# MAC-VO/MAC-VO

Hardware: AMD Instinct MI355X
Metric: stereo frames/sec at 640x480 (hot path: cost volume + lookup, keypoint selection, covariance, PGO) (higher is better)
Workload: dtype f32 via f16x2 (volume: fp32 operands row-scaled by powers of two and split into two fp16 pieces, three products, fp32 accumulate, scales undone exactly) + f32 (lookup/covariance) + f64 (PGO)

## Files before the change

mac-vo_amd/csrc/frontend_ops.hip:

```cpp
#include "common.h"
#include "randperm_dev.h"
#include "kp_draw_dev.h"
#include "match_cov_dev.h"
#include "pose_apply_dev.h"
#include "obs_filter_dev.h"
#include <math.h>

namespace {

__global__ __launch_bounds__(256) void frontend_epilogue_kernel(
    const float* __restrict__ flow, const float* __restrict__ logcov, int cov_is_log, int plane, float bl_fx,
    float bl_fx_sq, float* __restrict__ disparity, float* __restrict__ disparity_cov, float* __restrict__ depth,
    float* __restrict__ depth_cov, uint8_t* __restrict__ bad_mask, float* __restrict__ match_flow,
    float* __restrict__ match_cov) {
    MV_CHAIN_KERNEL_PRIO();
    const size_t lo = (size_t)blockIdx.y * plane;
    flow += 4 * lo; logcov += 4 * lo;
    if (disparity) disparity += lo;
    if (disparity_cov) disparity_cov += lo;
    if (depth) depth += lo;
    if (depth_cov) depth_cov += lo;
    if (bad_mask) bad_mask += lo;
    if (match_flow) match_flow += 2 * lo;
    if (match_cov) match_cov += 3 * lo;
// ... 170 lines not shown
    const float u = kp_uv[2 * n], v = kp_uv[2 * n + 1], d = depth_vals[(size_t)n * depth_stride];
    const float p[3] = {d, ((u - cx) * d) / fx, ((v - cy) * d) / fy};
    if (pos_Tc) { pos_Tc[3 * n] = p[0]; pos_Tc[3 * n + 1] = p[1]; pos_Tc[3 * n + 2] = p[2]; }
    if (pos_Tw) {
        float r[3];
        quat_act_f32(q, p, r);
        pos_Tw[3 * n] = r[0] + t[0]; pos_Tw[3 * n + 1] = r[1] + t[1]; pos_Tw[3 * n + 2] = r[2] + t[2];
    }
}

__global__ __launch_bounds__(256) void pose_apply_kernel(const float* __restrict__ pose, const float* __restrict__ pos_Tc,
                                                         const double* __restrict__ cov, int cap, mvLaneCounts cnt,
                                                         float* __restrict__ pos_Tw, double* __restrict__ rot,
                                                         double* __restrict__ cov_rot) {
    const int n = blockIdx.x * blockDim.x + threadIdx.x;
    const int lane = blockIdx.y;
    const int N = cnt.n[lane];
    {
        const size_t ln = (size_t)lane * cap;
        pose += 7 * lane;
        if (pos_Tc) pos_Tc += 3 * ln;
        if (pos_Tw) pos_Tw += 3 * ln;
        if (cov) cov += 9 * ln;
        if (cov_rot) cov_rot += 9 * ln;
        if (rot) rot += 9 * lane;
    }
    double R[9];
    mv_pose_rotation(pose, R);
    if (n == 0 && rot) {
#pragma unroll
        for (int i = 0; i < 9; ++i) rot[i] = R[i];
    }
    if (n >= N) return;
    mv_pose_apply_row(pose, R, n, pos_Tc, cov, pos_Tw, cov_rot);
}

__global__ __launch_bounds__(256) void map_points_kernel(const int64_t* __restrict__ uv, int N,
                                                          const float* __restrict__ depth, const float* __restrict__ depth_cov,
                                                          const float* __restrict__ image, int H, int W, float fx, float fy,
                                                          float cx, float cy, const float* __restrict__ pose,
                                                          float match_cov_default, float* __restrict__ out_uv,
                                                          float* __restrict__ out_d, float* __restrict__ out_sdd,
                                                          float* __restrict__ out_sigma, float* __restrict__ out_Tc,
                                                          float* __restrict__ out_Tw, uint8_t* __restrict__ out_color) {
    const int n = blockIdx.x * blockDim.x + threadIdx.x;
    if (n >= N) return;
    const int u = (int)uv[2 * n], v = (int)uv[2 * n + 1];
    const bool ok = u >= 0 && u < W && v >= 0 && v < H;
    const int i = ok ? v * W + u : 0;
    const float d = depth[i];
    const float uf = (float)u, vf = (float)v;
    out_uv[2 * n] = uf;
    out_uv[2 * n + 1] = vf;
    if (out_d) out_d[n] = d;
    if (out_sdd) out_sdd[n] = depth_cov ? depth_cov[i] : -1.f;
    if (out_sigma) { out_sigma[3 * n] = match_cov_default; out_sigma[3 * n + 1] = match_cov_default; out_sigma[3 * n + 2] = 0.f; }
    const float pc[3] = {d, ((uf - cx) * d) / fx, ((vf - cy) * d) / fy};
    if (out_Tc) { out_Tc[3 * n] = pc[0]; out_Tc[3 * n + 1] = pc[1]; out_Tc[3 * n + 2] = pc[2]; }
    if (out_Tw) {
        const float q[4] = {pose[3], pose[4], pose[5], pose[6]};
        float r[3];
        quat_act_f32(q, pc, r);
        out_Tw[3 * n] = r[0] + pose[0]; out_Tw[3 * n + 1] = r[1] + pose[1]; out_Tw[3 * n + 2] = r[2] + pose[2];
    }
    if (out_color && image) {
        const size_t plane = (size_t)H * W;
#pragma unroll
        for (int c = 0; c < 3; ++c) {
            const float x = image[c * plane + i] * 255.f;
            out_color[3 * n + c] = (uint8_t)(int)x;
        }
    }
}

__global__ __launch_bounds__(256) void obs_filter_kernel(const uint8_t* __restrict__ inbound,
                                                         const double* __restrict__ cov1,
                                                         const double* __restrict__ cov2,
                                                         const float* __restrict__ vals, int flags,
                                                         float min_depth, float max_depth, int cap, mvLaneCounts cnt,
                                                         uint8_t* __restrict__ valid, int32_t* __restrict__ count) {
    obs_filter_body(inbound, cov1, cov2, vals, flags, min_depth, max_depth, cap, cnt.n[blockIdx.x], blockIdx.x, gridDim.x, valid, count);
}

struct DrawArgs {
    const int32_t* count;
    int count_stride;
    float nomatch_c;
    const uint32_t* state_in;
    uint32_t* state_out;
    int k;
    int32_t cov_mods;
    int64_t* out_perm;
    int32_t* out_live;
};
struct DrawLds {
    mvrp::Scratch s;
    int32_t head[mvrp::NBUCKET];
    int32_t out[mvrp::MAX_HEAD];
};
template <int PM, int MODEL = MV_COV_MATCH, bool MODS = false, bool NOMATCH = false>
__global__ __launch_bounds__(256) void backend_front_kernel(const int32_t* __restrict__ cand, size_t cand_lane_stride, const int64_t* __restrict__ perm,
                                                            PermArg pa, int cap, mvLaneCounts cnt, int64_t* out_uv, TrackArgs a, float fx, float fy,
                                                            float cx, float cy, float* pos_Tc, const float* depth_map0, const float* depth_map1,
                                                            double* out_cov0, double* out_cov1, mvMatchCovParams cp, DrawArgs da) {
    __shared__ __attribute__((aligned(16))) char draw_raw[PM == 2 ? sizeof(DrawLds) : PM == 4 ? sizeof(mvkp::Scratch) : 16];
    DrawLds& D = *reinterpret_cast<DrawLds*>(draw_raw);
    const int lane = threadIdx.x & 63;
    const int n = blockIdx.x * 4 + (threadIdx.x >> 6);
    const int set = blockIdx.y, pl = blockIdx.z;
    int N;
    if constexpr (PM == 2) {
        const int64_t n_cand = da.count[(size_t)pl * da.count_stride];
        const bool adv = blockIdx.x == 0 && blockIdx.y == 0;
        N = mv_randperm_head_wg(da.state_in + (size_t)pl * mvrp::MT_STRIDE, adv ? da.state_out + (size_t)pl * mvrp::MT_STRIDE : nullptr, n_cand, da.k,
                                D.out, D.s, D.head);
        __syncthreads();
        if (adv) {
            for (int i = threadIdx.x; i < N; i += 256) da.out_perm[(size_t)pl * cap + i] = D.out[i];
            if (threadIdx.x == 0) { da.out_live[2 * pl] = N; da.out_live[2 * pl + 1] = (int32_t)n_cand; }
        }
    } else if constexpr (PM == 3) {
        if (da.count) {
            const int c = da.count[(size_t)pl * da.count_stride];
            N = c < 0 ? 0 : (c > cap ? cap : c);
        } else {
            N = cnt.n[pl];
        }
        if (da.out_live && blockIdx.x == 0 && blockIdx.y == 0 && threadIdx.x == 0) { da.out_live[2 * pl] = N; da.out_live[2 * pl + 1] = N; }
    } else if constexpr (PM == 4) {
        N = cnt.n[pl];
        const bool adv = blockIdx.x == 0 && blockIdx.y == 0;
        mv_kp_random_wg(da.state_in + (size_t)pl * mvrp::MT_STRIDE, adv ? da.state_out + (size_t)pl * mvrp::MT_STRIDE : nullptr, da.k,
                        *reinterpret_cast<mvkp::Scratch*>(draw_raw));
    } else {
        N = cnt.n[pl];
    }
    if (n < N) {
        int u0, v0;
        if constexpr (PM <= 2) {
            const int32_t* cand_l = cand + (size_t)pl * cand_lane_stride;
            const long pi = PM == 2 ? (long)D.out[n] : PM == 1 ? (long)pa.idx[n] : (long)perm[(size_t)pl * cap + n];
            const int lin = cand_l[pi];
            u0 = lin % a.W;
            v0 = lin / a.W;
        } else if constexpr (PM == 3) {
            const int64_t* kp = perm + 2 * ((size_t)pl * cap + n);
            u0 = (int)kp[0];
            v0 = (int)kp[1];
        } else if constexpr (PM == 4) {
            mvkp::row_of(reinterpret_cast<mvkp::Scratch*>(draw_raw)->w, da.k, n, a.H, a.W, pa.idx[0], u0, v0);
        } else {
            mvkp::grid_row(mvkp::Grid{pa.idx[0], 0, pa.idx[1], pa.idx[2], pa.idx[3]}, n, u0, v0);
        }
        TrackArgs al = a;
        track_lane_offsets(al, pl, cap);
        const size_t ln = (size_t)pl * cap;
        float u, v, suu, svv, suv;
        if (set == 0) {
            if (lane == 0) {
                if (PM != 3 || out_uv != perm) {
                    out_uv[2 * (ln + n) + 0] = u0;
                    out_uv[2 * (ln + n) + 1] = v0;
                }
                kp_track_one(n, u0, v0, al.match_flow, al.match_cov, al.depth0, al.disp0, al.sdisp0, al.sdd0, al.depth1, al.disp1, al.sdisp1, al.sdd1,
                             al.H, al.W, al.edge, al.match_cov_default, al.out_kp0, al.out_kp1, al.out_inbound, al.out_vals, (size_t)gridDim.z * cap,
                             nullptr, nullptr);
                al.out_sigma0[3 * n + 2] = 0.f;
                const float uf = (float)u0, vf = (float)v0, d = al.out_vals[n];
                float* pt = pos_Tc + 3 * (ln + n);
                pt[0] = d;
                pt[1] = ((uf - cx) * d) / fx;
                pt[2] = ((vf - cy) * d) / fy;
            }
            u = (float)u0; v = (float)v0;
            suu = a.match_cov_default; svv = a.match_cov_default; suv = 0.f;
        } else {
            const int plane = al.H * al.W;
            const bool ok0 = u0 >= 0 && u0 < al.W && v0 >= 0 && v0 < al.H;
            const int i0 = ok0 ? v0 * al.W + u0 : 0;
            u = (float)u0 + al.match_flow[i0];
            v = (float)v0 + al.match_flow[plane + i0];
            if constexpr (NOMATCH) {
                if (lane == 0) { al.out_sigma1[3 * n] = -1.f; al.out_sigma1[3 * n + 1] = -1.f; al.out_sigma1[3 * n + 2] = -1.f; }
                const bool inb = ok0 && (u < (float)(al.W - al.edge)) && (u > (float)al.edge) && (v < (float)(al.H - al.edge)) && (v > (float)al.edge);
                const bool have_var = al.sdd1 != nullptr;
                const float var = have_var && inb ? al.sdd1[(int)v * al.W + (int)u] : 0.f;
                const mvcov::CovSet S1{depth_map1, nullptr, nullptr, nullptr, nullptr, out_cov1, nullptr, nullptr};
                mvcov::match_cov_wave_vals<MODEL, MODS, true>(S1, cp, cap, pl, n, u, v, da.nomatch_c, da.nomatch_c, 0.f, da.cov_mods, a.sdd1, var, have_var);
                return;
            }
            suu = al.match_cov ? al.match_cov[i0] : -1.f;
            svv = al.match_cov ? al.match_cov[plane + i0] : -1.f;
            suv = al.match_cov ? al.match_cov[2 * plane + i0] : -1.f;
            if (lane == 0) al.out_sigma1[3 * n + 2] = suv;
        }
        const mvcov::CovSet S{set ? depth_map1 : depth_map0, nullptr, set ? a.out_sigma1 : a.out_sigma0, nullptr, nullptr, set ? out_cov1 : out_cov0,
                              nullptr, nullptr};
        if constexpr (MODEL == MV_COV_MATCH && !MODS)
            mvcov::match_cov_wave_vals(S, cp, cap, pl, n, u, v, suu, svv, suv);
        else
            mvcov::match_cov_wave_vals<MODEL, MODS>(S, cp, cap, pl, n, u, v, suu, svv, suv, da.cov_mods, set ? a.sdd1 : a.sdd0);
    }
}

template <int PM, typename... Args>
void launch_backend_front(int model, int32_t mods, bool nomatch, float nomatch_c, dim3 grid, hipStream_t st, DrawArgs da, Args... args) {
    const bool m = mods != 0;
    da.cov_mods = mods;
    if constexpr (PM >= 3) if (nomatch) {
        da.nomatch_c = nomatch_c;
        if (model == MV_COV_MATCH && !m)
            hipLaunchKernelGGL((backend_front_kernel<PM, MV_COV_MATCH, false, true>), grid, dim3(256), 0, st, args..., da);
        else if (model == MV_COV_MATCH)
            hipLaunchKernelGGL((backend_front_kernel<PM, MV_COV_MATCH, true, true>), grid, dim3(256), 0, st, args..., da);
        else if (model == MV_COV_GMM && !m)
            hipLaunchKernelGGL((backend_front_kernel<PM, MV_COV_GMM, false, true>), grid, dim3(256), 0, st, args..., da);
        else if (model == MV_COV_GMM)
            hipLaunchKernelGGL((backend_front_kernel<PM, MV_COV_GMM, true, true>), grid, dim3(256), 0, st, args..., da);
        else if (!m)
            hipLaunchKernelGGL((backend_front_kernel<PM, MV_COV_NONE, false, true>), grid, dim3(256), 0, st, args..., da);
        else
            hipLaunchKernelGGL((backend_front_kernel<PM, MV_COV_NONE, true, true>), grid, dim3(256), 0, st, args..., da);
        return;
    }
    if (model == MV_COV_MATCH && !m)
        hipLaunchKernelGGL((backend_front_kernel<PM>), grid, dim3(256), 0, st, args..., da);
    else if (model == MV_COV_MATCH)
        hipLaunchKernelGGL((backend_front_kernel<PM, MV_COV_MATCH, true>), grid, dim3(256), 0, st, args..., da);
    else if (model == MV_COV_GMM && !m)
        hipLaunchKernelGGL((backend_front_kernel<PM, MV_COV_GMM, false>), grid, dim3(256), 0, st, args..., da);
    else if (model == MV_COV_GMM)
        hipLaunchKernelGGL((backend_front_kernel<PM, MV_COV_GMM, true>), grid, dim3(256), 0, st, args..., da);
    else if (!m)
        hipLaunchKernelGGL((backend_front_kernel<PM, MV_COV_NONE, false>), grid, dim3(256), 0, st, args..., da);
    else
        hipLaunchKernelGGL((backend_front_kernel<PM, MV_COV_NONE, true>), grid, dim3(256), 0, st, args..., da);
}

template <typename... Args>
void launch_backend_front_pm(int pm, Args... args) {
    switch (pm) {
        case 1: return launch_backend_front<1>(args...);
        case 0: return launch_backend_front<0>(args...);
        case 2: return launch_backend_front<2>(args...);
        case 3: return launch_backend_front<3>(args...);
        case 4: return launch_backend_front<4>(args...);
        case 5: return launch_backend_front<5>(args...);
    }
}

}

extern "C" int mv_frontend_epilogue_lanes(const float* flow, const float* logcov, int cov_is_log, int H, int W,
                                          float bl_fx, float bl_fx_sq, float* disparity, float* disparity_cov,
                                          float* depth, float* depth_cov, uint8_t* bad_mask, float* match_flow,
                                          float* match_cov, int lanes, mvStream_t stream) {
    MV_CHECK_ARG(flow && H > 0 && W > 0 && lanes >= 1 && lanes <= MV_MAX_LANES);
    const int plane = H * W;
    const int blocks = min(mv_ceil_div(plane, 256), 2048);
    const bool no_d = !disparity_cov && !depth_cov, no_m = match_flow && !match_cov;
    MV_CHECK_ARG(logcov || (no_d && !match_cov));
    if (!logcov || no_d || no_m) {
        const dim3 grid(blocks, lanes);
#define MV_EPI_PARTIAL(D, M)                                                                                                                             \
    hipLaunchKernelGGL((frontend_epilogue_partial_kernel<D, M>), grid, dim3(256), 0, (hipStream_t)stream, flow, logcov, cov_is_log, plane, bl_fx, bl_fx_sq, \
                       disparity, disparity_cov, depth, depth_cov, bad_mask, match_flow, match_cov)
        if (!logcov || (no_d && !match_cov)) MV_EPI_PARTIAL(false, false);
        else if (no_d) MV_EPI_PARTIAL(false, true);
        else MV_EPI_PARTIAL(true, false);
#undef MV_EPI_PARTIAL
        return mv_launch_status();
    }
    hipLaunchKernelGGL(frontend_epilogue_kernel, dim3(blocks, lanes), dim3(256), 0, (hipStream_t)stream, flow, logcov,
                       cov_is_log, plane, bl_fx, bl_fx_sq, disparity, disparity_cov, depth, depth_cov, bad_mask,
                       match_flow, match_cov);
    return mv_launch_status();
}

extern "C" int mv_frontend_epilogue(const float* flow, const float* logcov, int cov_is_log, int H, int W,
                                    float bl_fx, float bl_fx_sq, float* disparity, float* disparity_cov, float* depth,
                                    float* depth_cov, uint8_t* bad_mask, float* match_flow, float* match_cov,
                                    mvStream_t stream) {
    return mv_frontend_epilogue_lanes(flow, logcov, cov_is_log, H, W, bl_fx, bl_fx_sq, disparity, disparity_cov, depth,
                                      depth_cov, bad_mask, match_flow, match_cov, 1, stream);
// ... 276 lines not shown
```

mac-vo_amd/csrc/match_cov_dev.h:

```cpp
#pragma once
#include "common.h"
#include <math.h>

namespace mvcov {

constexpr int MAX_K = 31;
constexpr int MAX_TAPS_PER_LANE = (MAX_K * MAX_K + 63) / 64;

__device__ __forceinline__ float clamp_min_nanprop(float x, float m) { return (x < m) ? m : x; }

struct CovSet {
    const float* depth_map;
    const float* kp_uv;
    float* flow_cov;
    const float* depth_cov;
    const double* rot;
    double* out_cov;
    double* out_cov_rot;
    float* out_stats;
};

__device__ __forceinline__ void apply_modifiers(double c[9], int32_t mods) {
#pragma unroll
    for (int s = 0; s < 4; ++s) {
        const int k = (mods >> (4 * s)) & 15;
        if (k == MV_COVMOD_DIAG) {
            c[1] = 0.0; c[2] = 0.0; c[3] = 0.0; c[5] = 0.0; c[6] = 0.0; c[7] = 0.0;
        } else if (k == MV_COVMOD_NORMALIZE) {
            const double det = (c[0] * (c[4] * c[8] - c[5] * c[7]) - c[1] * (c[3] * c[8] - c[5] * c[6])) + c[2] * (c[3] * c[7] - c[4] * c[6]);
#pragma unroll
            for (int i = 0; i < 9; ++i) c[i] = c[i] / det;
        }
    }
}

template <bool MODS>
__device__ __forceinline__ void store_cov(double c[9], int32_t mods, const double* rot, double* out_cov, double* out_cov_rot, float* out_stats,
                                          int n, float mu, float var) {
    if constexpr (MODS) apply_modifiers(c, mods);
    double* o = out_cov + (size_t)n * 9;
#pragma unroll
    for (int i = 0; i < 9; ++i) o[i] = c[i];
    if (out_cov_rot && rot) {
        double R[9], t[9];
#pragma unroll
        for (int i = 0; i < 9; ++i) R[i] = rot[i];
#pragma unroll
        for (int i = 0; i < 3; ++i)
#pragma unroll
            for (int j = 0; j < 3; ++j)
                t[3 * i + j] = (R[3 * i] * c[j] + R[3 * i + 1] * c[3 + j]) + R[3 * i + 2] * c[6 + j];
        double* orot = out_cov_rot + (size_t)n * 9;
#pragma unroll
        for (int i = 0; i < 3; ++i)
#pragma unroll
            for (int j = 0; j < 3; ++j)
                orot[3 * i + j] = (t[3 * i] * R[3 * j] + t[3 * i + 1] * R[3 * j + 1]) + t[3 * i + 2] * R[3 * j + 2];
    }
    if (out_stats) {
        out_stats[2 * n] = mu;
        out_stats[2 * n + 1] = var;
    }
}

template <int MODEL = MV_COV_MATCH, bool MODS = false, bool NOMATCH = false>
__device__ __forceinline__ void match_cov_wave_vals(const CovSet& S, const mvMatchCovParams& p, int cap, int pl, int n, float u, float v,
                                                    float suu, float svv, float suv, int32_t mods = 0,
                                                    const float* depth_cov_map_all = nullptr ,
                                                    float var_given = 0.f, bool have_var = false ) {
    const int lane = threadIdx.x & 63;
    const size_t ln = (size_t)pl * cap;
    const float* __restrict__ depth_map = S.depth_map + (size_t)pl * p.H * p.W;
    float* __restrict__ flow_cov = S.flow_cov + 3 * ln;
    const float* __restrict__ depth_cov = S.depth_cov ? S.depth_cov + ln : nullptr;
    const double* __restrict__ rot = S.rot ? S.rot + 9 * pl : nullptr;
    double* __restrict__ out_cov = S.out_cov + 9 * ln;
    double* __restrict__ out_cov_rot = S.out_cov_rot ? S.out_cov_rot + 9 * ln : nullptr;
    float* __restrict__ out_stats = S.out_stats ? S.out_stats + 2 * ln : nullptr;

    if constexpr (MODEL == MV_COV_NONE) {
        if (lane == 0) {
            if constexpr (!NOMATCH) {
                flow_cov[3 * n] = suu;
                flow_cov[3 * n + 1] = svv;
            }
            double c[9] = {1.0, 0.0, 0.0, 0.0, 1.0, 0.0, 0.0, 0.0, 1.0};
            store_cov<MODS>(c, mods, rot, out_cov, out_cov_rot, out_stats, n, __builtin_nanf(""), __builtin_nanf(""));
        }
        return;
    }
    const float* __restrict__ depth_cov_map = MODEL == MV_COV_GMM ? depth_cov_map_all + (size_t)pl * p.H * p.W : nullptr;

    const int iu = (int)u, iv = (int)v;
    if constexpr (!NOMATCH) {
        suu = clamp_min_nanprop(suu, p.min_flow_cov_sq);
        svv = clamp_min_nanprop(svv, p.min_flow_cov_sq);
        if (lane == 0) {
            flow_cov[3 * n] = suu;
            flow_cov[3 * n + 1] = svv;
        }
    }
    bool patch_var;
    if constexpr (NOMATCH) patch_var = !have_var; else patch_var = p.use_patch_var;

    const float det = suu * svv - suv * suv;
    const float m00 = -0.5f * (svv / det), m01 = -0.5f * (-suv / det), m11 = -0.5f * (suu / det);
    const float cnorm = (2.f * 3.14159265358979323846f) * sqrtf(det);

    const int K = p.kernel_size, h = K >> 1, taps = K * K;
    float z[MAX_TAPS_PER_LANE], kv[MAX_TAPS_PER_LANE];
    float zc[MODEL == MV_COV_GMM ? MAX_TAPS_PER_LANE : 1];
    float ksum = 0.f;
#pragma unroll
    for (int r = 0; r < MAX_TAPS_PER_LANE; ++r) {
        const int idx = r * 64 + lane;
        z[r] = 0.f;
        kv[r] = 0.f;
        if constexpr (MODEL == MV_COV_GMM) zc[r] = 0.f;
        if (idx < taps) {
            const int a = idx / K, b = idx - a * K;
            int yy = iv + (a - h), xx = iu + (b - h);
            yy = min(max(yy, 0), p.H - 1);
            xx = min(max(xx, 0), p.W - 1);
            z[r] = depth_map[yy * p.W + xx];
            if constexpr (MODEL == MV_COV_GMM) zc[r] = depth_cov_map[yy * p.W + xx] + z[r] * z[r];
            const float x0 = (float)(a - h), x1 = (float)(b - h);
            const float q = (x0 * m00) * x0 + 2.f * ((x0 * m01) * x1) + (x1 * m11) * x1;
            kv[r] = expf(q) / cnorm;
            ksum += kv[r];
        }
    }
    ksum = wave_sum(ksum);

    float mu = 0.f, var;
    if constexpr (MODEL == MV_COV_GMM) {
        float psum = 0.f;
#pragma unroll
        for (int r = 0; r < MAX_TAPS_PER_LANE; ++r) {
            kv[r] = kv[r] / ksum;
            if (kv[r] < 1e-3f) kv[r] = 0.f;
            psum += kv[r];
        }
        psum = wave_sum(psum);
        float e2 = 0.f;
#pragma unroll
        for (int r = 0; r < MAX_TAPS_PER_LANE; ++r) {
            kv[r] = kv[r] / psum;
            mu += z[r] * kv[r];
            e2 += zc[r] * kv[r];
        }
        mu = wave_sum(mu);
        e2 = wave_sum(e2);
        if constexpr (NOMATCH) var = patch_var ? (e2 - mu * mu) / 2.f : var_given;
        else var = patch_var ? (e2 - mu * mu) / 2.f : depth_cov[n];
    } else {
#pragma unroll
        for (int r = 0; r < MAX_TAPS_PER_LANE; ++r) {
            kv[r] = kv[r] / ksum;
            mu += kv[r] * z[r];
        }
        mu = wave_sum(mu);

        if (patch_var) {
            var = 0.f;
#pragma unroll
            for (int r = 0; r < MAX_TAPS_PER_LANE; ++r) {
                const float d = z[r] - mu;
                var += kv[r] * (d * d);
            }
            var = wave_sum(var);
        } else {
            if constexpr (NOMATCH) var = var_given; else var = depth_cov[n];
        }
        var = clamp_min_nanprop(var, p.min_depth_cov);
    }

    if (lane == 0) {
        const float du = u - p.cx, dv = v - p.cy;
        const float fx2 = p.fx * p.fx, fy2 = p.fy * p.fy, fxy = p.fx * p.fy;
        const float d2 = mu * mu;
        const float sxx = (((du * du) * var) + (d2 * suu) + (suu * var)) / fx2;
        const float syy = (((dv * dv) * var) + (d2 * svv) + (svv * var)) / fy2;
        const float szz = var;
        const float sxy = (((du * dv) * var) + (d2 + var) * suv) / fxy;
        const float sxz = (var * du) / p.fx;
        const float syz = (var * dv) / p.fy;
        double c[9] = {szz, sxz, syz, sxz, sxx, sxy, syz, sxy, syy};
        if constexpr (MODS) apply_modifiers(c, mods);
        double* o = out_cov + (size_t)n * 9;
#pragma unroll
        for (int i = 0; i < 9; ++i) o[i] = c[i];
        if (out_cov_rot && rot) {
            double R[9], t[9];
#pragma unroll
            for (int i = 0; i < 9; ++i) R[i] = rot[i];
#pragma unroll
            for (int i = 0; i < 3; ++i)
#pragma unroll
                for (int j = 0; j < 3; ++j)
                    t[3 * i + j] = (R[3 * i] * c[j] + R[3 * i + 1] * c[3 + j]) + R[3 * i + 2] * c[6 + j];
            double* orot = out_cov_rot + (size_t)n * 9;
#pragma unroll
            for (int i = 0; i < 3; ++i)
#pragma unroll
                for (int j = 0; j < 3; ++j)
                    orot[3 * i + j] = (t[3 * i] * R[3 * j] + t[3 * i + 1] * R[3 * j + 1]) + t[3 * i + 2] * R[3 * j + 2];
        }
        if (out_stats) {
            out_stats[2 * n] = mu;
            out_stats[2 * n + 1] = var;
        }
    }
}


template <int MODEL = MV_COV_MATCH, bool MODS = false>
__device__ __forceinline__ void match_cov_wave(const CovSet& S, const mvMatchCovParams& p, int cap, int pl, int n, int32_t mods = 0,
                                               const float* depth_cov_map = nullptr) {
    const size_t ln = (size_t)pl * cap;
    const float* __restrict__ kp_uv = S.kp_uv + 2 * ln;
    const float* __restrict__ flow_cov = S.flow_cov + 3 * ln;
    match_cov_wave_vals<MODEL, MODS>(S, p, cap, pl, n, kp_uv[2 * n], kp_uv[2 * n + 1], flow_cov[3 * n], flow_cov[3 * n + 1], flow_cov[3 * n + 2],
                                     mods, depth_cov_map);
}

template <int MODEL, bool MODS>
__device__ __forceinline__ void match_cov_wave_nomatch(const CovSet& S, const mvMatchCovParams& p, int cap, int pl, int n, float c, int32_t mods,
                                                       const float* depth_cov_map) {
    const size_t ln = (size_t)pl * cap;
    const float* __restrict__ kp_uv = S.kp_uv + 2 * ln;
    const bool have = S.depth_cov != nullptr;
    const float var = have ? S.depth_cov[ln + n] : 0.f;
    match_cov_wave_vals<MODEL, MODS, true>(S, p, cap, pl, n, kp_uv[2 * n], kp_uv[2 * n + 1], c, c, 0.f, mods, depth_cov_map, var, have);
}

}
```

mac-vo_amd/csrc/randperm.hip:

```cpp
#include "common.h"
#include "randperm_dev.h"
#include <vector>

int mv_randperm_heads_emulated_state(uint32_t* state, const int64_t* n, int calls, int k, int threads, int64_t* out);

namespace {

__global__ __launch_bounds__(1024) void randperm_head_kernel(uint32_t* __restrict__ state, const int32_t* __restrict__ n_dev, int n_stride, int k, int cap,
                                                             int64_t* __restrict__ out, int32_t* __restrict__ n_sel, int nsel_stride) {
    __shared__ mvrp::Scratch s;
    __shared__ int32_t head[mvrp::NBUCKET];
    const int l = blockIdx.x;
    uint32_t* const st = state + (size_t)l * mvrp::MT_STRIDE;
    const int m = mv_randperm_head_wg(st, st, (int64_t)n_dev[(size_t)l * n_stride], k, out + (size_t)l * cap, s, head);
    if (threadIdx.x == 0) n_sel[(size_t)l * nsel_stride] = m;
}

}

extern "C" int mv_randperm_state_words(void) { return mvrp::MT_STRIDE; }
extern "C" int mv_randperm_max_head(void) { return mvrp::MAX_HEAD; }

extern "C" int mv_mt19937_seed(uint64_t seed, uint32_t* state_host) {
    MV_CHECK_ARG(state_host);
    mvrp::mt_seed((uint32_t)(seed & 0xffffffffull), state_host);
    return MV_OK;
}

extern "C" int mv_randperm_head_lanes(uint32_t* state, const int32_t* n_dev, int n_stride, int lanes, int k, int cap, int64_t* out_perm, int32_t* out_n_sel,
                                      int n_sel_stride, mvStream_t stream) {
    MV_CHECK_ARG(state && n_dev && out_perm && out_n_sel && lanes >= 1 && n_stride >= 1 && n_sel_stride >= 1);
    MV_CHECK_ARG(k >= 0 && k <= cap);
    if (k > mvrp::MAX_HEAD) return MV_ERR_UNSUPPORTED;
    hipLaunchKernelGGL(randperm_head_kernel, dim3(lanes), dim3(1024), 0, (hipStream_t)stream, state, n_dev, n_stride, k, cap, out_perm, out_n_sel, n_sel_stride);
    return mv_launch_status();
}

extern "C" int mv_randperm_heads_emulated(uint64_t seed, const int64_t* n, int calls, int k, int threads, int64_t* out) {
    std::vector<uint32_t> state(mvrp::MT_STRIDE);
    mvrp::mt_seed((uint32_t)(seed & 0xffffffffull), state.data());
    return mv_randperm_heads_emulated_state(state.data(), n, calls, k, threads, out);
}

int mv_randperm_heads_emulated_state(uint32_t* state, const int64_t* n, int calls, int k, int threads, int64_t* out) {
    using namespace mvrp;
    MV_CHECK_ARG(state && n && out && calls >= 0 && k >= 0 && threads >= 1 && threads <= 4096);
    if (k > MAX_HEAD) return MV_ERR_UNSUPPORTED;
    std::vector<int32_t> head(NBUCKET);
    Scratch* s = new Scratch;
    const int nt = threads;
#define MV_RP_ALL(call) for (int tid = 0; tid < nt; ++tid) { call; }
    for (int c = 0; c < calls; ++c) {
        MV_CHECK_ARG(n[c] >= 0 && n[c] < ((int64_t)1 << 31));
        const Plan pl = plan_of(n[c], k);
        MV_RP_ALL(phase_clear(head.data(), tid, nt));
        if (pl.advance > 0) {
            for (int i = 0; i < MT_N; ++i) s->mt[0][i] = state[i];
            int pos = (int)state[MT_N], cur = 0;
            int64_t produced = 0, rem = pl.advance;
            while (rem > 0) {
                if (pos == MT_N) {
                    MV_RP_ALL(phase_step(s->mt[cur], s->mt[cur ^ 1], tid, nt));
                    cur ^= 1;
                    pos = 0;
                }
                const int take = (int)(rem < MT_N - pos ? rem : MT_N - pos);
                if (produced < pl.swaps) MV_RP_ALL(phase_draws(s->mt[cur], pos, take, produced, pl, s->t, tid, nt));
                pos += take;
                produced += take;
                rem -= take;
            }
            for (int i = 0; i < MT_N; ++i) state[i] = s->mt[cur][i];
            state[MT_N] = (uint32_t)pos;
        }
        MV_RP_ALL(phase_insert(*s, head.data(), pl, tid, nt));
        MV_RP_ALL(phase_link(*s, head.data(), pl, tid, nt));
        MV_RP_ALL(phase_emit(*s, pl, out + (size_t)c * k, tid, nt));
    }
#undef MV_RP_ALL
    delete s;
    return MV_OK;
}
```

mac-vo_amd/csrc/randperm_dev.h:

```cpp
#pragma once
#include <stdint.h>

#if defined(__HIPCC__)
#define MV_RP_FN __host__ __device__ __forceinline__
#else
#define MV_RP_FN inline
#endif

namespace mvrp {

constexpr int MT_N = 624;
constexpr int MT_STRIDE = 640;
constexpr int MAX_HEAD = 512;
constexpr int NBUCKET = 1024;

struct Scratch {
    uint32_t mt[2][MT_N];
    int32_t t[MAX_HEAD], nxt[MAX_HEAD], ptr[MAX_HEAD], hit[MAX_HEAD];
};

MV_RP_FN uint32_t mt_f(uint32_t a, uint32_t b) {
    const uint32_t y = (a & 0x80000000u) | (b & 0x7fffffffu);
    return (y >> 1) ^ ((b & 1u) ? 0x9908b0dfu : 0u);
}
// ... 17 lines not shown

inline void mt_seed(uint32_t seed, uint32_t* state ) {
    state[0] = seed;
    for (int i = 1; i < MT_N; ++i) state[i] = 1812433253u * (state[i - 1] ^ (state[i - 1] >> 30)) + (uint32_t)i;
    state[MT_N] = MT_N;
    for (int i = MT_N + 1; i < MT_STRIDE; ++i) state[i] = 0;
}

struct Plan {
    int64_t n;
    int swaps, m;
    int64_t advance;
};
MV_RP_FN Plan plan_of(int64_t n, int k) {
    Plan p;
    p.n = n;
    p.m = (int)(n < k ? (n < 0 ? 0 : n) : k);
    p.swaps = n >= 1 ? (int)(k < n - 1 ? k : n - 1) : 0;
    p.advance = n >= 1 ? n - 1 : 0;
    return p;
}

MV_RP_FN void phase_step(const uint32_t* o, uint32_t* nw, int tid, int nt) {
    for (int k = tid; k < MT_N; k += nt) nw[k] = mt_step_word(o, k);
}

MV_RP_FN void phase_draws(const uint32_t* x, int pos, int take, int64_t produced, const Plan& pl, int32_t* t, int tid, int nt) {
    for (int j = tid; j < take; j += nt) {
        const int64_t g = produced + j;
        if (g >= pl.swaps) break;
        t[g] = (int32_t)(g + (int64_t)(mt_temper(x[pos + j]) % (uint32_t)(pl.n - g)));
    }
}

MV_RP_FN void phase_clear(int32_t* head, int tid, int nt) {
    for (int b = tid; b < NBUCKET; b += nt) head[b] = -1;
}

#if defined(__HIP_DEVICE_COMPILE__)
#define MV_RP_XCHG(p, v) atomicExch((p), (v))
#else
static inline int32_t mv_rp_xchg_host(int32_t* p, int32_t v) { const int32_t o = *p; *p = v; return o; }
#define MV_RP_XCHG(p, v) mv_rp_xchg_host((p), (v))
#endif

MV_RP_FN void phase_insert(Scratch& s, int32_t* head, const Plan& pl, int tid, int nt) {
    for (int j = tid; j < pl.m; j += nt) {
        if (j < pl.swaps) s.nxt[j] = MV_RP_XCHG(&head[s.t[j] & (NBUCKET - 1)], j);
        else s.t[j] = j;
    }
}

MV_RP_FN int32_t prev_of(const Scratch& s, const int32_t* head, int i, int32_t p) {
    int32_t best = -1;
    for (int32_t e = head[p & (NBUCKET - 1)]; e >= 0; e = s.nxt[e])
        if (e < i && s.t[e] == p && e > best) best = e;
    return best;
}

MV_RP_FN void phase_link(Scratch& s, const int32_t* head, const Plan& pl, int tid, int nt) {
    for (int i = tid; i < pl.m; i += nt) {
        s.ptr[i] = prev_of(s, head, i, i);
        s.hit[i] = s.t[i] == i ? -2 : prev_of(s, head, i, s.t[i]);
    }
}

MV_RP_FN int32_t root_of(const Scratch& s, int32_t i) {
    while (s.ptr[i] >= 0) i = s.ptr[i];
    return i;
}

template <typename T>
MV_RP_FN void phase_emit(const Scratch& s, const Plan& pl, T* out, int tid, int nt) {
    for (int i = tid; i < pl.m; i += nt) {
        const int32_t h = s.hit[i];
        out[i] = (T)(h == -2 ? root_of(s, i) : (h >= 0 ? root_of(s, h) : s.t[i]));
    }
}

}

#if defined(__HIPCC__)
template <typename T>
__device__ __forceinline__ int mv_randperm_head_wg(const uint32_t* __restrict__ state_in, uint32_t* state_out, int64_t n, int k, T* out, mvrp::Scratch& s,
                                                   int32_t* head) {
    using namespace mvrp;
    const int tid = threadIdx.x, nt = blockDim.x;
    const Plan pl = plan_of(n, k);
    phase_clear(head, tid, nt);
    if (pl.advance > 0 || state_out) {
        for (int i = tid; i < MT_N; i += nt) s.mt[0][i] = state_in[i];
        int pos = (int)state_in[MT_N];
        __syncthreads();
        int cur = 0;
        int64_t produced = 0;
        const int64_t total = state_out ? pl.advance : (int64_t)pl.swaps;
        int64_t rem = total;
        while (rem > 0) {
            if (pos == MT_N) {
                phase_step(s.mt[cur], s.mt[cur ^ 1], tid, nt);
                __syncthreads();
                cur ^= 1;
                pos = 0;
            }
            const int take = (int)(rem < MT_N - pos ? rem : MT_N - pos);
            if (produced < pl.swaps) phase_draws(s.mt[cur], pos, take, produced, pl, s.t, tid, nt);
            pos += take;
            produced += take;
            rem -= take;
        }
        if (state_out) {
            for (int i = tid; i < MT_N; i += nt) state_out[i] = s.mt[cur][i];
            if (tid == 0) state_out[MT_N] = (uint32_t)pos;
        }
    }
    __syncthreads();
    phase_insert(s, head, pl, tid, nt);
    __syncthreads();
    phase_link(s, head, pl, tid, nt);
    __syncthreads();
    phase_emit(s, pl, out, tid, nt);
    return pl.m;
}
#endif
```

Baseline: 7564.

## Issue front-kernel pixel and window loads early and spread them across lanes

In the backend front kernel, lane 0 no longer does a serial chain of pixel reads through kp_track_one. Each lane now loads one source or tracked pixel value, and the values are broadcast with readlane. The covariance window taps and Gaussian weights move into separate request and weights phases that run before the per-set branching, so global loads are in flight earlier. The randperm head also prefetches the Mersenne Twister state and count into registers before the plan is computed. The aim is to shorten the latency-bound dependent load chain, at the cost of more registers and duplicated inbound logic. A standalone timing probe script is added as well.

```diff
diff --git a/mac-vo_amd/csrc/frontend_ops.hip b/mac-vo_amd/csrc/frontend_ops.hip
--- a/mac-vo_amd/csrc/frontend_ops.hip
+++ b/mac-vo_amd/csrc/frontend_ops.hip
@@ -276,6 +276,27 @@
     obs_filter_body(inbound, cov1, cov2, vals, flags, min_depth, max_depth, cap, cnt.n[blockIdx.x], blockIdx.x, gridDim.x, valid, count);
 }
 
+enum { FS_FLOW_U, FS_FLOW_V, FS_SUU, FS_SVV, FS_SUV, FS_DEPTH, FS_DISP, FS_SDISP, FS_SDD };
+__device__ __forceinline__ float lane_value(float x, int k) { return __int_as_float(__builtin_amdgcn_readlane(__float_as_int(x), k)); }
+__device__ __forceinline__ float front_source_pixel(const TrackArgs& al, int lane, int i0, int plane) {
+    const float* p = al.match_flow;
+    int off = i0;
+    if (lane == FS_FLOW_V) off = plane + i0;
+    if (lane >= FS_SUU && lane <= FS_SUV && al.match_cov) { p = al.match_cov; off = (lane - FS_SUU) * plane + i0; }
+    if (lane == FS_DEPTH) p = al.depth0;
+    if (lane == FS_DISP && al.disp0) p = al.disp0;
+    if (lane == FS_SDISP && al.sdisp0) p = al.sdisp0;
+    if (lane == FS_SDD && al.sdd0) p = al.sdd0;
+    return p[off];
+}
+__device__ __forceinline__ float front_tracked_pixel(const TrackArgs& al, int lane, int i1) {
+    const float* p = al.depth1;
+    if (lane == 1 && al.disp1) p = al.disp1;
+    if (lane == 2 && al.sdisp1) p = al.sdisp1;
+    if (lane == 3 && al.sdd1) p = al.sdd1;
+    return p[i1];
+}
+
 struct DrawArgs {
     const int32_t* count;
     int count_stride;
@@ -304,10 +325,10 @@
     const int set = blockIdx.y, pl = blockIdx.z;
     int N;
     if constexpr (PM == 2) {
-        const int64_t n_cand = da.count[(size_t)pl * da.count_stride];
+        int64_t n_cand;
         const bool adv = blockIdx.x == 0 && blockIdx.y == 0;
-        N = mv_randperm_head_wg(da.state_in + (size_t)pl * mvrp::MT_STRIDE, adv ? da.state_out + (size_t)pl * mvrp::MT_STRIDE : nullptr, n_cand, da.k,
-                                D.out, D.s, D.head);
+        N = mv_randperm_head_wg(da.state_in + (size_t)pl * mvrp::MT_STRIDE, adv ? da.state_out + (size_t)pl * mvrp::MT_STRIDE : nullptr,
+                                da.count + (size_t)pl * da.count_stride, n_cand, da.k, D.out, D.s, D.head);
         __syncthreads();
         if (adv) {
             for (int i = threadIdx.x; i < N; i += 256) da.out_perm[(size_t)pl * cap + i] = D.out[i];
@@ -349,51 +370,82 @@
         TrackArgs al = a;
         track_lane_offsets(al, pl, cap);
         const size_t ln = (size_t)pl * cap;
-        float u, v, suu, svv, suv;
+        const int plane = al.H * al.W;
+        const bool ok0 = u0 >= 0 && u0 < al.W && v0 >= 0 && v0 < al.H;
+        const int i0 = ok0 ? v0 * al.W + u0 : 0;
+        const float x0 = front_source_pixel(al, lane, i0, plane);
+        if constexpr (NOMATCH) if (set == 1) {
+            const float u = (float)u0 + lane_value(x0, FS_FLOW_U);
+            const float v = (float)v0 + lane_value(x0, FS_FLOW_V);
+            const bool inb = ok0 && (u < (float)(al.W - al.edge)) && (u > (float)al.edge) && (v < (float)(al.H - al.edge)) && (v > (float)al.edge);
+            const bool have_var = al.sdd1 != nullptr;
+            const float var1 = (have_var ? al.sdd1 : al.depth1)[inb ? (int)v * al.W + (int)u : 0];
+            mvcov::CovWindow<MODEL> w;
+            mvcov::cov_window_request<MODEL>(depth_map1, a.sdd1, cp, pl, u, v, w);
+            float suu = da.nomatch_c, svv = da.nomatch_c;
+            mvcov::cov_window_weights<MODEL, true>(cp, suu, svv, 0.f, w);
+            if (lane == 0) { al.out_sigma1[3 * n] = -1.f; al.out_sigma1[3 * n + 1] = -1.f; al.out_sigma1[3 * n + 2] = -1.f; }
+            const float var = have_var && inb ? var1 : 0.f;
+            const mvcov::CovSet S1{depth_map1, nullptr, nullptr, nullptr, nullptr, out_cov1, nullptr, nullptr};
+            mvcov::match_cov_wave_finish<MODEL, MODS, true>(S1, cp, cap, pl, n, u, v, suu, svv, 0.f, da.cov_mods, var, have_var, w);
+            return;
+        }
+        float u = (float)u0, v = (float)v0;
+        float suu = a.match_cov_default, svv = a.match_cov_default, suv = 0.f;
+        if (set == 1) {
+            u = (float)u0 + lane_value(x0, FS_FLOW_U);
+            v = (float)v0 + lane_value(x0, FS_FLOW_V);
+            suu = al.match_cov ? lane_value(x0, FS_SUU) : -1.f;
+            svv = al.match_cov ? lane_value(x0, FS_SVV) : -1.f;
+            suv = al.match_cov ? lane_value(x0, FS_SUV) : -1.f;
+        }
+        mvcov::CovWindow<MODEL> w;
+        mvcov::cov_window_request<MODEL>(set ? depth_map1 : depth_map0, set ? a.sdd1 : a.sdd0, cp, pl, u, v, w);
+        mvcov::cov_window_weights<MODEL, false>(cp, suu, svv, suv, w);
         if (set == 0) {
+            const float u1 = (float)u0 + lane_value(x0, FS_FLOW_U);
+            const float v1 = (float)v0 + lane_value(x0, FS_FLOW_V);
+            const bool inb = ok0 && (u1 < (float)(al.W - al.edge)) && (u1 > (float)al.edge) && (v1 < (float)(al.H - al.edge)) && (v1 > (float)al.edge);
+            const int i1 = inb ? (int)v1 * al.W + (int)u1 : 0;
+            const float x1 = front_tracked_pixel(al, lane, i1);
+            const float d = lane_value(x0, FS_DEPTH);
+            const float t_disp = lane_value(x0, FS_DISP), t_sdisp = lane_value(x0, FS_SDISP), t_sdd = lane_value(x0, FS_SDD);
+            const float m_uu = lane_value(x0, FS_SUU), m_vv = lane_value(x0, FS_SVV), m_uv = lane_value(x0, FS_SUV);
+            const float d1 = lane_value(x1, 0), t_disp1 = lane_value(x1, 1), t_sdisp1 = lane_value(x1, 2), t_sdd1 = lane_value(x1, 3);
             if (lane == 0) {
                 if (PM != 3 || out_uv != perm) {
                     out_uv[2 * (ln + n) + 0] = u0;
                     out_uv[2 * (ln + n) + 1] = v0;
                 }
-                kp_track_one(n, u0, v0, al.match_flow, al.match_cov, al.depth0, al.disp0, al.sdisp0, al.sdd0, al.depth1, al.disp1, al.sdisp1, al.sdd1,
-                             al.H, al.W, al.edge, al.match_cov_default, al.out_kp0, al.out_kp1, al.out_inbound, al.out_vals, (size_t)gridDim.z * cap,
-                             nullptr, nullptr);
+                if (al.out_kp0) { al.out_kp0[2 * n] = (float)u0; al.out_kp0[2 * n + 1] = (float)v0; }
+                al.out_kp1[2 * n] = u1;
+                al.out_kp1[2 * n + 1] = v1;
+                al.out_inbound[n] = inb;
+                const size_t vs = (size_t)gridDim.z * cap;
+                float* o = al.out_vals + n;
+                o[0 * vs] = d;
+                o[1 * vs] = al.disp0 ? t_disp : -1.f;
+                o[2 * vs] = al.sdisp0 ? t_sdisp : -1.f;
+                o[3 * vs] = al.sdd0 ? t_sdd : -1.f;
+                o[4 * vs] = inb ? d1 : 0.f;
+                o[5 * vs] = inb ? (al.disp1 ? t_disp1 : -1.f) : 0.f;
+                o[6 * vs] = inb ? (al.sdisp1 ? t_sdisp1 : -1.f) : 0.f;
+                o[7 * vs] = inb ? (al.sdd1 ? t_sdd1 : -1.f) : 0.f;
+                o[8 * vs] = al.match_cov ? m_uu : -1.f;
+                o[9 * vs] = al.match_cov ? m_vv : -1.f;
+                o[10 * vs] = al.match_cov ? m_uv : -1.f;
                 al.out_sigma0[3 * n + 2] = 0.f;
-                const float uf = (float)u0, vf = (float)v0, d = al.out_vals[n];
                 float* pt = pos_Tc + 3 * (ln + n);
                 pt[0] = d;
-                pt[1] = ((uf - cx) * d) / fx;
-                pt[2] = ((vf - cy) * d) / fy;
+                pt[1] = ((u - cx) * d) / fx;
+                pt[2] = ((v - cy) * d) / fy;
             }
-            u = (float)u0; v = (float)v0;
-            suu = a.match_cov_default; svv = a.match_cov_default; suv = 0.f;
-        } else {
-            const int plane = al.H * al.W;
-            const bool ok0 = u0 >= 0 && u0 < al.W && v0 >= 0 && v0 < al.H;
-            const int i0 = ok0 ? v0 * al.W + u0 : 0;
-            u = (float)u0 + al.match_flow[i0];
-            v = (float)v0 + al.match_flow[plane + i0];
-            if constexpr (NOMATCH) {
-                if (lane == 0) { al.out_sigma1[3 * n] = -1.f; al.out_sigma1[3 * n + 1] = -1.f; al.out_sigma1[3 * n + 2] = -1.f; }
-                const bool inb = ok0 && (u < (float)(al.W - al.edge)) && (u > (float)al.edge) && (v < (float)(al.H - al.edge)) && (v > (float)al.edge);
-                const bool have_var = al.sdd1 != nullptr;
-                const float var = have_var && inb ? al.sdd1[(int)v * al.W + (int)u] : 0.f;
-                const mvcov::CovSet S1{depth_map1, nullptr, nullptr, nullptr, nullptr, out_cov1, nullptr, nullptr};
-                mvcov::match_cov_wave_vals<MODEL, MODS, true>(S1, cp, cap, pl, n, u, v, da.nomatch_c, da.nomatch_c, 0.f, da.cov_mods, a.sdd1, var, have_var);
-                return;
-            }
-            suu = al.match_cov ? al.match_cov[i0] : -1.f;
-            svv = al.match_cov ? al.match_cov[plane + i0] : -1.f;
-            suv = al.match_cov ? al.match_cov[2 * plane + i0] : -1.f;
-            if (lane == 0) al.out_sigma1[3 * n + 2] = suv;
+        } else if (lane == 0) {
+            al.out_sigma1[3 * n + 2] = suv;
         }
         const mvcov::CovSet S{set ? depth_map1 : depth_map0, nullptr, set ? a.out_sigma1 : a.out_sigma0, nullptr, nullptr, set ? out_cov1 : out_cov0,
                               nullptr, nullptr};
-        if constexpr (MODEL == MV_COV_MATCH && !MODS)
-            mvcov::match_cov_wave_vals(S, cp, cap, pl, n, u, v, suu, svv, suv);
-        else
-            mvcov::match_cov_wave_vals<MODEL, MODS>(S, cp, cap, pl, n, u, v, suu, svv, suv, da.cov_mods, set ? a.sdd1 : a.sdd0);
+        mvcov::match_cov_wave_finish<MODEL, MODS, false>(S, cp, cap, pl, n, u, v, suu, svv, suv, da.cov_mods, 0.f, false, w);
     }
 }
 
diff --git a/mac-vo_amd/csrc/match_cov_dev.h b/mac-vo_amd/csrc/match_cov_dev.h
--- a/mac-vo_amd/csrc/match_cov_dev.h
+++ b/mac-vo_amd/csrc/match_cov_dev.h
@@ -63,14 +63,82 @@
     }
 }
 
-template <int MODEL = MV_COV_MATCH, bool MODS = false, bool NOMATCH = false>
-__device__ __forceinline__ void match_cov_wave_vals(const CovSet& S, const mvMatchCovParams& p, int cap, int pl, int n, float u, float v,
-                                                    float suu, float svv, float suv, int32_t mods = 0,
-                                                    const float* depth_cov_map_all = nullptr ,
-                                                    float var_given = 0.f, bool have_var = false ) {
+struct TapWalk {
+    int a, b, q, rem;
+    __device__ __forceinline__ TapWalk(int lane, int K) : a(lane / K), b(lane - (lane / K) * K), q(64 / K), rem(64 - (64 / K) * K) {}
+    __device__ __forceinline__ void next(int K) {
+        a += q;
+        b += rem;
+        if (b >= K) { b -= K; ++a; }
+    }
+};
+
+template <int MODEL>
+struct CovWindow {
+    float z[MAX_TAPS_PER_LANE];
+    float c[MODEL == MV_COV_GMM ? MAX_TAPS_PER_LANE : 1];
+    float kv[MAX_TAPS_PER_LANE];
+    float ksum;
+};
+
+template <int MODEL>
+__device__ __forceinline__ void cov_window_request(const float* depth_map_all, const float* depth_cov_map_all, const mvMatchCovParams& p, int pl, float u,
+                                                   float v, CovWindow<MODEL>& w) {
+    if constexpr (MODEL != MV_COV_NONE) {
+        const int lane = threadIdx.x & 63;
+        const float* __restrict__ depth_map = depth_map_all + (size_t)pl * p.H * p.W;
+        const float* __restrict__ depth_cov_map = MODEL == MV_COV_GMM ? depth_cov_map_all + (size_t)pl * p.H * p.W : nullptr;
+        const int iu = (int)u, iv = (int)v;
+        const int K = p.kernel_size, h = K >> 1;
+        TapWalk t(lane, K);
+#pragma unroll
+        for (int r = 0; r < MAX_TAPS_PER_LANE; ++r, t.next(K)) {
+            const int a = t.a, b = t.b;
+            int yy = iv + (a - h), xx = iu + (b - h);
+            yy = min(max(yy, 0), p.H - 1);
+            xx = min(max(xx, 0), p.W - 1);
+            w.z[r] = depth_map[yy * p.W + xx];
+            if constexpr (MODEL == MV_COV_GMM) w.c[r] = depth_cov_map[yy * p.W + xx];
+        }
+    }
+}
+
+template <int MODEL, bool NOMATCH>
+__device__ __forceinline__ void cov_window_weights(const mvMatchCovParams& p, float& suu, float& svv, float suv, CovWindow<MODEL>& w) {
+    if constexpr (MODEL != MV_COV_NONE) {
+        const int lane = threadIdx.x & 63;
+        if constexpr (!NOMATCH) {
+            suu = clamp_min_nanprop(suu, p.min_flow_cov_sq);
+            svv = clamp_min_nanprop(svv, p.min_flow_cov_sq);
+        }
+        const float det = suu * svv - suv * suv;
+        const float m00 = -0.5f * (svv / det), m01 = -0.5f * (-suv / det), m11 = -0.5f * (suu / det);
+        const float cnorm = (2.f * 3.14159265358979323846f) * sqrtf(det);
+
+        const int K = p.kernel_size, h = K >> 1, taps = K * K;
+        float ksum = 0.f;
+        TapWalk t(lane, K);
+#pragma unroll
+        for (int r = 0; r < MAX_TAPS_PER_LANE; ++r, t.next(K)) {
+            const int idx = r * 64 + lane;
+            w.kv[r] = 0.f;
+            if (idx < taps) {
+                const int a = t.a, b = t.b;
+                const float x0 = (float)(a - h), x1 = (float)(b - h);
+                const float q = (x0 * m00) * x0 + 2.f * ((x0 * m01) * x1) + (x1 * m11) * x1;
+                w.kv[r] = expf(q) / cnorm;
+                ksum += w.kv[r];
+            }
+        }
+        w.ksum = wave_sum(ksum);
+    }
+}
+
+template <int MODEL, bool MODS, bool NOMATCH>
+__device__ __forceinline__ void match_cov_wave_finish(const CovSet& S, const mvMatchCovParams& p, int cap, int pl, int n, float u, float v, float suu,
+                                                      float svv, float suv, int32_t mods, float var_given, bool have_var, CovWindow<MODEL>& w) {
     const int lane = threadIdx.x & 63;
     const size_t ln = (size_t)pl * cap;
-    const float* __restrict__ depth_map = S.depth_map + (size_t)pl * p.H * p.W;
     float* __restrict__ flow_cov = S.flow_cov + 3 * ln;
     const float* __restrict__ depth_cov = S.depth_cov ? S.depth_cov + ln : nullptr;
     const double* __restrict__ rot = S.rot ? S.rot + 9 * pl : nullptr;
@@ -89,12 +157,7 @@
         }
         return;
     }
-    const float* __restrict__ depth_cov_map = MODEL == MV_COV_GMM ? depth_cov_map_all + (size_t)pl * p.H * p.W : nullptr;
-
-    const int iu = (int)u, iv = (int)v;
     if constexpr (!NOMATCH) {
-        suu = clamp_min_nanprop(suu, p.min_flow_cov_sq);
-        svv = clamp_min_nanprop(svv, p.min_flow_cov_sq);
         if (lane == 0) {
             flow_cov[3 * n] = suu;
             flow_cov[3 * n + 1] = svv;
@@ -103,34 +166,17 @@
     bool patch_var;
     if constexpr (NOMATCH) patch_var = !have_var; else patch_var = p.use_patch_var;
 
-    const float det = suu * svv - suv * suv;
-    const float m00 = -0.5f * (svv / det), m01 = -0.5f * (-suv / det), m11 = -0.5f * (suu / det);
-    const float cnorm = (2.f * 3.14159265358979323846f) * sqrtf(det);
-
-    const int K = p.kernel_size, h = K >> 1, taps = K * K;
-    float z[MAX_TAPS_PER_LANE], kv[MAX_TAPS_PER_LANE];
+    const int taps = p.kernel_size * p.kernel_size;
+    float* z = w.z;
+    float* kv = w.kv;
     float zc[MODEL == MV_COV_GMM ? MAX_TAPS_PER_LANE : 1];
-    float ksum = 0.f;
 #pragma unroll
     for (int r = 0; r < MAX_TAPS_PER_LANE; ++r) {
-        const int idx = r * 64 + lane;
-        z[r] = 0.f;
-        kv[r] = 0.f;
-        if constexpr (MODEL == MV_COV_GMM) zc[r] = 0.f;
-        if (idx < taps) {
-            const int a = idx / K, b = idx - a * K;
-            int yy = iv + (a - h), xx = iu + (b - h);
-            yy = min(max(yy, 0), p.H - 1);
-            xx = min(max(xx, 0), p.W - 1);
-            z[r] = depth_map[yy * p.W + xx];
-            if constexpr (MODEL == MV_COV_GMM) zc[r] = depth_cov_map[yy * p.W + xx] + z[r] * z[r];
-            const float x0 = (float)(a - h), x1 = (float)(b - h);
-            const float q = (x0 * m00) * x0 + 2.f * ((x0 * m01) * x1) + (x1 * m11) * x1;
-            kv[r] = expf(q) / cnorm;
-            ksum += kv[r];
-        }
-    }
-    ksum = wave_sum(ksum);
+        const bool live = r * 64 + lane < taps;
+        z[r] = live ? z[r] : 0.f;
+        if constexpr (MODEL == MV_COV_GMM) zc[r] = live ? w.c[r] + z[r] * z[r] : 0.f;
+    }
+    const float ksum = w.ksum;
 
     float mu = 0.f, var;
     if constexpr (MODEL == MV_COV_GMM) {
@@ -213,6 +259,17 @@
     }
 }
 
+template <int MODEL = MV_COV_MATCH, bool MODS = false, bool NOMATCH = false>
+__device__ __forceinline__ void match_cov_wave_vals(const CovSet& S, const mvMatchCovParams& p, int cap, int pl, int n, float u, float v,
+                                                    float suu, float svv, float suv, int32_t mods = 0,
+                                                    const float* depth_cov_map_all = nullptr ,
+                                                    float var_given = 0.f, bool have_var = false ) {
+    CovWindow<MODEL> w;
+    cov_window_request<MODEL>(S.depth_map, depth_cov_map_all, p, pl, u, v, w);
+    cov_window_weights<MODEL, NOMATCH>(p, suu, svv, suv, w);
+    match_cov_wave_finish<MODEL, MODS, NOMATCH>(S, p, cap, pl, n, u, v, suu, svv, suv, mods, var_given, have_var, w);
+}
+
 
 template <int MODEL = MV_COV_MATCH, bool MODS = false>
 __device__ __forceinline__ void match_cov_wave(const CovSet& S, const mvMatchCovParams& p, int cap, int pl, int n, int32_t mods = 0,
diff --git a/mac-vo_amd/csrc/randperm.hip b/mac-vo_amd/csrc/randperm.hip
--- a/mac-vo_amd/csrc/randperm.hip
+++ b/mac-vo_amd/csrc/randperm.hip
@@ -12,7 +12,8 @@
     __shared__ int32_t head[mvrp::NBUCKET];
     const int l = blockIdx.x;
     uint32_t* const st = state + (size_t)l * mvrp::MT_STRIDE;
-    const int m = mv_randperm_head_wg(st, st, (int64_t)n_dev[(size_t)l * n_stride], k, out + (size_t)l * cap, s, head);
+    int64_t n;
+    const int m = mv_randperm_head_wg(st, st, n_dev + (size_t)l * n_stride, n, k, out + (size_t)l * cap, s, head);
     if (threadIdx.x == 0) n_sel[(size_t)l * nsel_stride] = m;
 }
 
diff --git a/mac-vo_amd/csrc/randperm_dev.h b/mac-vo_amd/csrc/randperm_dev.h
--- a/mac-vo_amd/csrc/randperm_dev.h
+++ b/mac-vo_amd/csrc/randperm_dev.h
@@ -123,15 +123,30 @@
 
 #if defined(__HIPCC__)
 template <typename T>
-__device__ __forceinline__ int mv_randperm_head_wg(const uint32_t* __restrict__ state_in, uint32_t* state_out, int64_t n, int k, T* out, mvrp::Scratch& s,
-                                                   int32_t* head) {
+__device__ __forceinline__ int mv_randperm_head_wg(const uint32_t* state_in, uint32_t* state_out, const int32_t* n_dev, int64_t& n_out, int k, T* out,
+                                                   mvrp::Scratch& s, int32_t* head) {
     using namespace mvrp;
     const int tid = threadIdx.x, nt = blockDim.x;
+    constexpr int EARLY = 3;
+    uint32_t early[EARLY];
+#pragma unroll
+    for (int r = 0; r < EARLY; ++r) {
+        const int i = tid + r * nt;
+        early[r] = state_in[i < MT_N ? i : MT_N];
+    }
+    const uint32_t pos_in = state_in[MT_N];
+    const int64_t n = *n_dev;
+    n_out = n;
+    phase_clear(head, tid, nt);
     const Plan pl = plan_of(n, k);
-    phase_clear(head, tid, nt);
     if (pl.advance > 0 || state_out) {
-        for (int i = tid; i < MT_N; i += nt) s.mt[0][i] = state_in[i];
-        int pos = (int)state_in[MT_N];
+#pragma unroll
+        for (int r = 0; r < EARLY; ++r) {
+            const int i = tid + r * nt;
+            if (i < MT_N) s.mt[0][i] = early[r];
+        }
+        for (int i = tid + EARLY * nt; i < MT_N; i += nt) s.mt[0][i] = state_in[i];
+        int pos = (int)pos_in;
         __syncthreads();
         int cur = 0;
         int64_t produced = 0;
diff --git a/profiles/probes/front_alone.py b/profiles/probes/front_alone.py
--- /dev/null
+++ b/profiles/probes/front_alone.py
@@ -0,0 +1,65 @@
+#!/usr/bin/env python
+import argparse
+import ctypes as C
+import os
+import statistics
+import sys
+
+sys.path.insert(0, os.path.dirname(os.path.dirname(os.path.dirname(os.path.abspath(__file__)))))
+import torch
+
+from macvo_amd import _lib as L
+from macvo_amd import ops
+
+
+def main():
+    ap = argparse.ArgumentParser()
+    ap.add_argument("--reps", type=int, default=400)
+    ap.add_argument("--rounds", type=int, default=5)
+    a = ap.parse_args()
+    dev = torch.device("cuda:0")
+    lib = L.load()
+    print("library:", os.environ.get("MACVO_HIP_LIB") or L.LIB_PATH)
+    g = torch.Generator().manual_seed(0)
+    H, W, k, cap, n_cand = 480, 640, 200, 256, 4550
+    r = lambda *s: torch.rand(*s, generator=g).to(dev)
+    flow, cov = (r(1, 2, H, W) - 0.5) * 8, r(1, 3, H, W) + 0.05
+    cov[:, 2] *= 0.01
+    maps = [r(1, H, W) * 9 + 0.5 for _ in range(8)]
+    vv = torch.randint(32, H - 32, (n_cand,), generator=g)
+    uu = torch.randint(32, W - 32, (n_cand,), generator=g)
+    cand = (vv * W + uu).to(torch.int32).to(dev)
+    count = torch.tensor([n_cand], dtype=torch.int32, device=dev)
+    st = [ops.mt19937_state([3], dev), ops.mt19937_state([3], dev)]
+    z = lambda *s, dt=torch.float32: torch.zeros(s, dtype=dt, device=dev)
+    outs = [z(1, cap, dt=torch.int64), z(1, 2, dt=torch.int32), z(1, cap, 2, dt=torch.int64), z(1, cap, 2), z(1, cap, 2), z(1, cap, dt=torch.uint8),
+            z(11, 1, cap), z(1, cap, 3), z(1, cap, 3), z(1, cap, 3), z(1, cap, 9, dt=torch.float64), z(1, cap, 9, dt=torch.float64)]
+    cp = L.mvMatchCovParams(H, W, 31, 1, 320.0, 320.0, 320.0, 240.0, 0.0625, 0.05)
+    s = ops._stream()
+    calls = [0]
+
+    def launch():
+        i = calls[0] & 1
+        calls[0] += 1
+        L.check(lib.mv_backend_front_draw_lanes(cand.data_ptr(), n_cand, count.data_ptr(), 1, st[i].data_ptr(), st[i ^ 1].data_ptr(), k, 1, cap, flow.data_ptr(),
+                                                cov.data_ptr(), *[m.data_ptr() for m in maps], 32, 0.25, C.byref(cp), *[o.data_ptr() for o in outs], s),
+                "mv_backend_front_draw_lanes")
+
+    for _ in range(20):
+        launch()
+    torch.cuda.synchronize()
+    per = []
+    for _ in range(a.rounds):
+        e0, e1 = torch.cuda.Event(enable_timing=True), torch.cuda.Event(enable_timing=True)
+        e0.record()
+        for _ in range(a.reps):
+            launch()
+        e1.record()
+        torch.cuda.synchronize()
+        per.append(e0.elapsed_time(e1) * 1e3 / a.reps)
+    print(f"mv_backend_front_draw_lanes (backend_front_kernel<2, match>)  {statistics.median(per):7.2f} us  [{min(per):.2f} .. {max(per):.2f}]")
+    print("live rows / candidates of the last call:", outs[1][0].tolist(), " inbound:", int(outs[5].sum()))
+
+
+if __name__ == "__main__":
+    main()
```

Result: no change. 7593, median of 4 (+0.4%).
